# hila-chefer/Transformer-Explainability

Measured on AMD Instinct MI355X. Metric: relevance maps/sec (ViT-B/16 224^2, batch 64 per GPU, generate_LRP transformer_attribution), higher is better.
Workload: dtype f32 (3xbf16 split operands, 6 products, fp32 accumulate)

## Files before the change

### include/te_relprop.h

```cpp
#ifndef TE_RELPROP_H
#define TE_RELPROP_H

#include <stddef.h>
#include <stdint.h>

#ifdef __cplusplus
extern "C" {
#endif

typedef void* te_stream_t;
typedef uint16_t te_bf16_t;

enum {
  TE_OK = 0,
  TE_ERR_INVALID_ARG = -1,
  TE_ERR_WORKSPACE = -2,
  TE_ERR_UNSUPPORTED = -3,
  TE_ERR_NO_DEVICE = -4
};

enum { TE_VARIANT_OURS = 0, TE_VARIANT_LRP = 1, TE_IMPL_SIMPLE = 0x100 };

enum { TE_ROLLOUT_NORMALISE = 1, TE_ROLLOUT_CLS_FIXUP = 2, TE_ROLLOUT_ROW0 = 4 };

// ... 46 lines not shown
                       void* ws, size_t ws_bytes, te_stream_t stream);

size_t te_add_relprop_deferred_workspace_bytes(int64_t B, int64_t n);
int te_add_relprop_deferred_f32(const float* R, const float* X0, const float* X1, float* a, float* b, float* fac,
                                int64_t B, int64_t n, int64_t x1_batch_stride,
                                void* ws, size_t ws_bytes, te_stream_t stream);

size_t te_add_bcast_relprop_workspace_bytes(int64_t B, int64_t H, int64_t N);
int te_add_bcast_relprop_f32(const float* R, const float* X0, const float* mask, float* out0,
                             float* out1, int64_t B, int64_t H, int64_t N, int variant,
                             void* ws, size_t ws_bytes, te_stream_t stream);

int te_add_bcast_relprop_deferred_f32(const float* R, const float* X0, const float* mask, float* a, float* out1,
                                      float* fac, int64_t B, int64_t H, int64_t N,
                                      void* ws, size_t ws_bytes, te_stream_t stream);

int te_clone_relprop_f32(const float* R0, const float* R1, const float* R2, const float* X,
                         float* out, int64_t n, te_stream_t stream);

int te_clone_relprop_scaled_f32(const float* R0, const float* s0, int64_t s0_stride,
                                const float* R1, const float* s1, int64_t s1_stride,
                                const float* R2, const float* s2, int64_t s2_stride,
                                const float* X, float* out, int64_t B, int64_t n, te_stream_t stream);

int te_index_select_relprop_f32(const float* R, const float* X, float* out,
                                int64_t B, int64_t N, int64_t C, int64_t index, te_stream_t stream);

int te_gradcam_headmean_f32(const float* grad, const float* cam, float* out,
                            int64_t B, int64_t H, int64_t N, te_stream_t stream);

size_t te_rollout_workspace_bytes(int64_t L, int64_t B, int64_t N);
size_t te_rollout_row0_workspace_bytes(int64_t B, int64_t N);
int te_rollout_f32(const float* cams, int64_t L, int64_t start_layer, int64_t B, int64_t N,
                   int flags, float* joint, void* ws, size_t ws_bytes, te_stream_t stream);

#define TE_X6_TILE_AUTO 0
#define TE_X6_TILE_128 1
#define TE_X6_TILE_256 2
#define TE_X6_TILE_128x128 3
#define TE_X6_TEST_DROP_HANDOVER 0x200
#define TE_X6_WHOLE_TILES 0x10000
#define TE_X6_TEST_SMALL_GRID 0x4000
#define TE_X6_X_PLANES_SIGNED 0x20000
#define TE_X6_TILE_Z_SHIFT 10
#define TE_X6_TILE_C_SHIFT 12
#define TE_X6_PHASE_SPLIT 4
// ... 51 lines not shown
int te_attention_strided_supported(int64_t N, int64_t D);
size_t te_attention_backward_strided_workspace_bytes(int64_t B, int64_t H, int64_t N);
int te_attention_forward_strided_f32(const float* q, int64_t q_sb, int64_t q_sh, int64_t q_sn,
                                     const float* k, int64_t k_sb, int64_t k_sh, int64_t k_sn,
                                     const float* v, int64_t v_sb, int64_t v_sh, int64_t v_sn,
                                     const float* mask, float* z_qk, float* x_scaled, float* attn,
                                     float* out, int64_t o_sb, int64_t o_sh, int64_t o_sn,
                                     int64_t B, int64_t H, int64_t N, int64_t D, float scale, te_stream_t stream);
int te_attention_backward_strided_f32(const float* d_out, int64_t do_sb, int64_t do_sh, int64_t do_sn,
                                      const float* out, int64_t o_sb, int64_t o_sh, int64_t o_sn,
                                      const float* q, int64_t q_sb, int64_t q_sh, int64_t q_sn,
                                      const float* k, int64_t k_sb, int64_t k_sh, int64_t k_sn,
                                      const float* v, int64_t v_sb, int64_t v_sh, int64_t v_sn,
                                      const float* attn, float* d_attn,
                                      float* d_q, int64_t dq_sb, int64_t dq_sh, int64_t dq_sn,
                                      float* d_k, int64_t dk_sb, int64_t dk_sh, int64_t dk_sn,
                                      float* d_v, int64_t dv_sb, int64_t dv_sh, int64_t dv_sn,
                                      int64_t B, int64_t H, int64_t N, int64_t D, float scale, int need_qk,
                                      void* ws, size_t ws_bytes, te_stream_t stream);

int te_layernorm_supported(int64_t C);
int te_layernorm_forward_f32(const float* x, const float* weight, const float* bias, float* y, float* mean, float* rstd,
                             int64_t T, int64_t C, float eps, te_stream_t stream);
int te_layernorm_backward_f32(const float* dy, const float* x, const float* weight, const float* mean, const float* rstd,
                              const float* add, float* dx, int64_t T, int64_t C, te_stream_t stream);
int te_gelu_forward_f32(const float* x, float* y, int64_t n, te_stream_t stream);
int te_gelu_backward_f32(const float* dy, const float* x, float* dx, int64_t n, te_stream_t stream);

int te_heatmap_f32(const float* maps, float* heat, float* fg_mask, int64_t B, int64_t g, int64_t scale,
                   int normalise, te_stream_t stream);

size_t te_seg_metrics_workspace_bytes(int64_t B, int64_t H, int64_t W);
int te_seg_metrics_f32(const float* heat, const float* fg_mask, const int64_t* labels, int64_t* counts, double* ap,
                       double* f1, int64_t B, int64_t H, int64_t W, void* ws, size_t ws_bytes, te_stream_t stream);

#define TE_MAPSIM_SSIM 1
size_t te_map_similarity_workspace_bytes(int64_t B, int64_t n);
int te_map_similarity_f32(const float* a, const float* b, int64_t* rank_sums, double* sim, int64_t B, int64_t n, int64_t H,
                          int64_t W, int flags, double data_range, void* ws, size_t ws_bytes, te_stream_t stream);

#define TE_RATIONALE_MAX_KS 16
#define TE_RATIONALE_CLAMP 1
size_t te_rationale_metrics_workspace_bytes(int64_t B, int64_t N, int64_t Wmax);
int te_rationale_metrics_f32(const float* scores, const int32_t* word_ids, const uint8_t* truth, float* word_scores,
                             int32_t* n_words, int32_t* order, int32_t* counts, double* soft, int64_t B, int64_t N,
                             int64_t Wmax, const int64_t* ks, int64_t n_ks, int flags, void* ws, size_t ws_bytes,
// ... 212 lines not shown
```

### transformer-explainability_amd/csrc/te_api.hip

```cpp
#include "te_common.h"

#include <string.h>

extern "C" int te_version(void) { return 800;  }

#ifndef TE_BUILD_ID
#define TE_BUILD_ID "unstamped"
#endif
extern "C" const char* te_build_id(void) { return TE_BUILD_ID; }

extern "C" const char* te_status_string(int status) {
  switch (status) {
    case TE_OK: return "ok";
    case TE_ERR_INVALID_ARG: return "invalid argument";
    case TE_ERR_WORKSPACE: return "workspace missing, misaligned or too small";
    case TE_ERR_UNSUPPORTED: return "shape not supported by the gfx950 kernels";
    case TE_ERR_NO_DEVICE: return "no gfx950 device visible";
    default: break;
  }
  if (status > 0) return hipGetErrorString((hipError_t)status);
  return "unknown status";
}

extern "C" int te_device_check(void) {
  int n = 0;
  if (hipGetDeviceCount(&n) != hipSuccess || n <= 0) return TE_ERR_NO_DEVICE;
  for (int d = 0; d < n; ++d) {
// ... 7 lines not shown
```

### transformer-explainability_amd/csrc/te_elementwise.hip

```cpp
#include <stdlib.h>

#include "te_common.h"

namespace {

constexpr int kThreads = 256;


template <typename V>
__device__ __forceinline__ V ld(const float* p) { return *reinterpret_cast<const V*>(p); }
template <typename V>
__device__ __forceinline__ void st(float* p, V v) { *reinterpret_cast<V*>(p) = v; }

__device__ __forceinline__ float ldx(const float* p) { return *p; }
__device__ __forceinline__ float ldx(const te_bf16_t* p) { return __uint_as_float((unsigned)*p << 16); }
template <typename V>
__device__ __forceinline__ V ldx4(const float* p) { return ld<V>(p); }
template <typename V>
__device__ __forceinline__ V ldx4(const te_bf16_t* p) { return V{ldx(p), ldx(p + 1), ldx(p + 2), ldx(p + 3)}; }
static inline bool vec_aligned(const float* p) { return te_aligned16(p); }
static inline bool vec_aligned(const te_bf16_t*) { return true; }

template <int VEC, typename TX>
__global__ __launch_bounds__(kThreads) void add_sums_kernel(
// ... 354 lines not shown
  const TX* x_ = X + b * n;
  float* o = out + b * n;
  const int64_t stride = (int64_t)gridDim.x * kThreads * VEC;
  for (int64_t i = ((int64_t)blockIdx.x * kThreads + threadIdx.x) * VEC; i < n; i += stride) {
    if constexpr (VEC == 4) {
      const f32x4 x = ldx4<f32x4>(x_ + i), a = ld<f32x4>(r0 + i), bq = ld<f32x4>(r1 + i);
      f32x4 c = {0.f, 0.f, 0.f, 0.f};
      if constexpr (NUM == 3) c = ld<f32x4>(r2 + i);
      f32x4 ov;
#pragma unroll
      for (int e = 0; e < 4; ++e) {
        const float ra = s0 ? a[e] * f0 : a[e], rb = s1 ? bq[e] * f1 : bq[e];
        float s = te_sd(ra, x[e]) + te_sd(rb, x[e]);
        if constexpr (NUM == 3) s = s + te_sd(s2 ? c[e] * f2 : c[e], x[e]);
        ov[e] = x[e] * s;
      }
      st<f32x4>(o + i, ov);
    } else {
      const float x = ldx(x_ + i);
      float s = te_sd(s0 ? r0[i] * f0 : r0[i], x) + te_sd(s1 ? r1[i] * f1 : r1[i], x);
      if constexpr (NUM == 3) s = s + te_sd(s2 ? r2[i] * f2 : r2[i], x);
      o[i] = x * s;
    }
  }
}

template <typename TX>
__global__ __launch_bounds__(kThreads) void index_select_kernel(
    const float* __restrict__ R, const TX* __restrict__ X, float* __restrict__ out,
    int64_t B, int64_t N, int64_t C, int64_t index) {
  const int64_t total = B * N * C;
  const int64_t stride = (int64_t)gridDim.x * kThreads;
  for (int64_t i = (int64_t)blockIdx.x * kThreads + threadIdx.x; i < total; i += stride) {
    const int64_t c = i % C;
    const int64_t nrow = (i / C) % N;
    const int64_t b = i / (C * N);
    float v = 0.0f;
    if (nrow == index) {
      const float x = ldx(X + i);
      v = x * te_sd(R[b * C + c], x);
    }
    out[i] = v;
  }
}

template <int VEC, typename TG>
// ... 385 lines not shown
                                    float* out, int64_t n, te_stream_t stream_) {
  return clone_relprop(R0, R1, R2, X, out, n, stream_);
}

extern "C" int te_clone_relprop_bf16(const float* R0, const float* R1, const float* R2, const te_bf16_t* X, float* out,
                                     int64_t n, te_stream_t stream_) {
  return clone_relprop(R0, R1, R2, X, out, n, stream_);
}

extern "C" int te_clone_relprop_scaled_f32(const float* R0, const float* s0, int64_t s0_stride, const float* R1,
                                           const float* s1, int64_t s1_stride, const float* R2, const float* s2,
                                           int64_t s2_stride, const float* X, float* out, int64_t B, int64_t n,
                                           te_stream_t stream_) {
  return clone_relprop_scaled(R0, s0, s0_stride, R1, s1, s1_stride, R2, s2, s2_stride, X, out, B, n, stream_);
}

extern "C" int te_clone_relprop_scaled_bf16(const float* R0, const float* s0, int64_t s0_stride, const float* R1,
                                            const float* s1, int64_t s1_stride, const float* R2, const float* s2,
                                            int64_t s2_stride, const te_bf16_t* X, float* out, int64_t B, int64_t n,
                                            te_stream_t stream_) {
  return clone_relprop_scaled(R0, s0, s0_stride, R1, s1, s1_stride, R2, s2, s2_stride, X, out, B, n, stream_);
}

namespace {
template <typename TX>
int index_select_relprop(const float* R, const TX* X, float* out, int64_t B, int64_t N, int64_t C, int64_t index,
                         te_stream_t stream_) {
  if (!R || !X || !out || B <= 0 || N <= 0 || C <= 0 || index < 0 || index >= N)
    return TE_ERR_INVALID_ARG;
  hipStream_t stream = (hipStream_t)stream_;
  int64_t blocks = te_ceil_div(B * N * C, (int64_t)kThreads * 4);
  if (blocks > 4096) blocks = 4096;
  index_select_kernel<<<dim3((unsigned)blocks), dim3(kThreads), 0, stream>>>(R, X, out, B, N, C, index);
  TE_RETURN_IF_LAUNCH_FAILED();
  return TE_OK;
}

}

extern "C" int te_index_select_relprop_f32(const float* R, const float* X, float* out, int64_t B,
                                           int64_t N, int64_t C, int64_t index, te_stream_t stream_) {
  return index_select_relprop(R, X, out, B, N, C, index, stream_);
}

extern "C" int te_index_select_relprop_bf16(const float* R, const te_bf16_t* X, float* out, int64_t B, int64_t N,
                                            int64_t C, int64_t index, te_stream_t stream_) {
// ... 57 lines not shown
```

### transformer-explainability_amd/csrc/te_norm_act.hip

```cpp
#include "te_common.h"

namespace {

constexpr int kThreads = 256;
constexpr int kRowsPerBlock = kThreads / 64;
constexpr int kMaxChunks = 8;

__device__ __forceinline__ float wave_sum_all(float v) {
#pragma unroll
  for (int off = 32; off > 0; off >>= 1) v = v + __shfl_xor(v, off, 64);
  return v;
}

template <int NV>
__global__ __launch_bounds__(kThreads) void ln_fwd_kernel(const float* __restrict__ x, const float* __restrict__ w,
                                                          const float* __restrict__ b, float* __restrict__ y,
                                                          float* __restrict__ mean, float* __restrict__ rstd, int64_t T,
                                                          int C, float eps) {
  const int lane = threadIdx.x & 63;
  const int64_t row = (int64_t)blockIdx.x * kRowsPerBlock + (threadIdx.x >> 6);
  if (row >= T) return;
  const int nc = C >> 2;
  const float* xr = x + row * C;
  f32x4 v[NV];
  float s = 0.0f;
#pragma unroll
  for (int i = 0; i < NV; ++i) {
    const int c = lane + 64 * i;
    v[i] = f32x4{0.f, 0.f, 0.f, 0.f};
    if (c < nc) v[i] = *reinterpret_cast<const f32x4*>(xr + (c << 2));
    s = s + ((v[i][0] + v[i][1]) + (v[i][2] + v[i][3]));
  }
  const float m = wave_sum_all(s) / (float)C;
  float q = 0.0f;
#pragma unroll
  for (int i = 0; i < NV; ++i) {
    const int c = lane + 64 * i;
    if (c < nc) {
#pragma unroll
      for (int e = 0; e < 4; ++e) {
        const float d = v[i][e] - m;
        q = q + d * d;
      }
    }
  }
  const float r = 1.0f / sqrtf(wave_sum_all(q) / (float)C + eps);
  float* yr = y + row * C;
#pragma unroll
  for (int i = 0; i < NV; ++i) {
    const int c = lane + 64 * i;
    if (c < nc) {
      const f32x4 wv = *reinterpret_cast<const f32x4*>(w + (c << 2));
      const f32x4 bv = b ? *reinterpret_cast<const f32x4*>(b + (c << 2)) : f32x4{0.f, 0.f, 0.f, 0.f};
// ... 96 lines not shown
  }
  return TE_OK;
}

}

extern "C" int te_layernorm_supported(int64_t C) { return (C >= 4 && C % 4 == 0 && C <= 64 * 4 * kMaxChunks) ? 1 : 0; }

extern "C" int te_layernorm_forward_f32(const float* x, const float* weight, const float* bias, float* y, float* mean,
                                        float* rstd, int64_t T, int64_t C, float eps, te_stream_t stream_) {
  if (!x || !weight || !y || !mean || !rstd || T <= 0) return TE_ERR_INVALID_ARG;
  if (!te_layernorm_supported(C) || (T + kRowsPerBlock - 1) / kRowsPerBlock > 0x7fffffff) return TE_ERR_UNSUPPORTED;
  if (!te_aligned16(x) || !te_aligned16(weight) || !te_aligned16(y) || (bias && !te_aligned16(bias))) return TE_ERR_UNSUPPORTED;
  hipStream_t stream = (hipStream_t)stream_;
  const dim3 grid((unsigned)((T + kRowsPerBlock - 1) / kRowsPerBlock)), blk(kThreads);
  const int rc = for_chunks(C, [&](auto nv) {
    ln_fwd_kernel<decltype(nv)::value><<<grid, blk, 0, stream>>>(x, weight, bias, y, mean, rstd, T, (int)C, eps);
  });
  if (rc != TE_OK) return rc;
  TE_RETURN_IF_LAUNCH_FAILED();
  return TE_OK;
}

extern "C" int te_layernorm_backward_f32(const float* dy, const float* x, const float* weight, const float* mean,
                                         const float* rstd, const float* add, float* dx, int64_t T, int64_t C,
                                         te_stream_t stream_) {
  if (!dy || !x || !weight || !mean || !rstd || !dx || T <= 0) return TE_ERR_INVALID_ARG;
  if (!te_layernorm_supported(C) || (T + kRowsPerBlock - 1) / kRowsPerBlock > 0x7fffffff) return TE_ERR_UNSUPPORTED;
  if (!te_aligned16(dy) || !te_aligned16(x) || !te_aligned16(weight) || !te_aligned16(dx) || (add && !te_aligned16(add)))
    return TE_ERR_UNSUPPORTED;
  hipStream_t stream = (hipStream_t)stream_;
  const dim3 grid((unsigned)((T + kRowsPerBlock - 1) / kRowsPerBlock)), blk(kThreads);
  const int rc = for_chunks(C, [&](auto nv) {
    ln_bwd_kernel<decltype(nv)::value><<<grid, blk, 0, stream>>>(dy, x, weight, mean, rstd, add, dx, T, (int)C);
  });
  if (rc != TE_OK) return rc;
  TE_RETURN_IF_LAUNCH_FAILED();
  return TE_OK;
}

extern "C" int te_gelu_forward_f32(const float* x, float* y, int64_t n, te_stream_t stream_) {
  if (!x || !y || n <= 0) return TE_ERR_INVALID_ARG;
  if (n % 4 || !te_aligned16(x) || !te_aligned16(y) || n / 4 / kThreads > 0x7ffffffe) return TE_ERR_UNSUPPORTED;
  const int64_t n4 = n / 4;
  gelu_fwd_kernel<<<dim3((unsigned)((n4 + kThreads - 1) / kThreads)), dim3(kThreads), 0, (hipStream_t)stream_>>>(x, y, n4);
  TE_RETURN_IF_LAUNCH_FAILED();
// ... 12 lines not shown
```

### transformer-explainability_amd/ops.py

```python
from __future__ import annotations

import contextlib
import os
from typing import Optional, Sequence, Tuple

import torch

from . import _lib
from ._lib import (TE_HEADMEAN_CLAMP, TE_HEADMEAN_ROW0, TE_IMPL_SIMPLE, TE_RATIONALE_CLAMP, TE_ROLLOUT_CLS_FIXUP,
                   TE_ROLLOUT_NORMALISE, TE_ROLLOUT_ROW0, TE_VARIANT_LRP, TE_VARIANT_OURS)
from ._lib import (TE_X6_PHASE_C, TE_X6_PHASE_SPLIT, TE_X6_PHASE_Z, TE_X6_TEST_DROP_HANDOVER,
                   TE_X6_TEST_SMALL_GRID, TE_X6_TILE_C_SHIFT, TE_X6_TILE_Z_SHIFT, TE_X6_WHOLE_TILES, TE_X6_X_PLANES_SIGNED)

Tensor = torch.Tensor
_VARIANTS = {"ours": TE_VARIANT_OURS, "lrp": TE_VARIANT_LRP}

FORCE_SIMPLE = False
KERNEL_TIMER = None
_NULL = contextlib.nullcontext()


def _timed(name: str, flops: float = 0.0, nbytes: float = 0.0):
    return _NULL if KERNEL_TIMER is None else KERNEL_TIMER(name, float(flops), float(nbytes))

# ... 805 lines not shown
                   "te_attention_backward_f32")
    return d_attn, d_qkv


def layernorm_supported(x: Tensor) -> bool:
    return (x.is_cuda and x.dtype == torch.float32 and x.dim() >= 2
            and bool(_lib.load().te_layernorm_supported(int(x.shape[-1]))))


def layernorm_forward(x: Tensor, weight: Tensor, bias: Optional[Tensor], eps: float) -> Tuple[Tensor, Tensor, Tensor]:
    x = _c(x)
    C = x.shape[-1]
    T = x.numel() // C
    y = torch.empty_like(x)
    mean = torch.empty((T,), dtype=torch.float32, device=x.device)
    rstd = torch.empty((T,), dtype=torch.float32, device=x.device)
    with _on_device(x) as lib, _timed("layernorm_forward", 0.0, 4.0 * 2 * T * C):
        _lib.check(lib.te_layernorm_forward_f32(_ptr(x), _ptr(_c(weight)), _ptr(_c(bias)) if bias is not None else None,
                                                _ptr(y), _ptr(mean), _ptr(rstd), T, C, float(eps), _stream(x)),
                   "te_layernorm_forward_f32")
    return y, mean, rstd


def layernorm_backward(dy: Tensor, x: Tensor, weight: Tensor, mean: Tensor, rstd: Tensor,
                       add: Optional[Tensor] = None) -> Tensor:
    dy, x = _c(dy), _c(x)
    C = x.shape[-1]
    T = x.numel() // C
    dx = torch.empty_like(x)
    with _on_device(x) as lib, _timed("layernorm_backward", 0.0, 4.0 * (3 + (add is not None)) * T * C):
        _lib.check(lib.te_layernorm_backward_f32(_ptr(dy), _ptr(x), _ptr(_c(weight)), _ptr(mean), _ptr(rstd),
                                                 _ptr(_c(add)) if add is not None else None, _ptr(dx), T, C, _stream(x)),
                   "te_layernorm_backward_f32")
    return dx


def gelu_forward(x: Tensor) -> Tensor:
    x = _c(x)
    y = torch.empty_like(x)
    with _on_device(x) as lib, _timed("gelu_forward", 0.0, 4.0 * 2 * x.numel()):
        _lib.check(lib.te_gelu_forward_f32(_ptr(x), _ptr(y), x.numel(), _stream(x)), "te_gelu_forward_f32")
    return y


X6_FUSE_GELU = os.environ.get("TE_X6_FUSE_GELU", "1") not in ("", "0")

# ... 124 lines not shown
    X = _c16(X) if bf else _c(X)
    sfx = "bf16" if bf else "f32"
    pairs = [_split_deferred(r) for r in Rs]
    Rs = [_c(r) for r, _ in pairs]
    scales = [sc for _, sc in pairs]
    for r in Rs:
        if r.numel() != X.numel():
            raise _lib.TeError("Clone.relprop: relevance / input size mismatch")
    out = torch.empty(X.shape, dtype=torch.float32, device=X.device)
    nb = 4.0 * X.numel() * (len(Rs) + 1) + X.element_size() * X.numel()
    if any(sc is not None for sc in scales):
        B = X.shape[0]
        sp = [(None, 0) if sc is None else (sc.data_ptr(), sc.stride(0)) for sc in scales] + [(None, 0)]
        with _on_device(X) as lib, _timed("clone", 0.0, nb):
            _lib.check(getattr(lib, "te_clone_relprop_scaled_" + sfx)(
                _ptr(Rs[0]), sp[0][0], sp[0][1], _ptr(Rs[1]), sp[1][0], sp[1][1], _ptr(Rs[2]) if len(Rs) == 3 else None,
                sp[2][0], sp[2][1], _ptr(X), _ptr(out), B, X.numel() // B, _stream(X)), "te_clone_relprop_scaled_" + sfx)
        return out
    with _on_device(X) as lib, _timed("clone", 0.0, nb):
        _lib.check(getattr(lib, "te_clone_relprop_" + sfx)(_ptr(Rs[0]), _ptr(Rs[1]), _ptr(Rs[2]) if len(Rs) == 3 else None,
                                                           _ptr(X), _ptr(out), X.numel(), _stream(X)),
                   "te_clone_relprop_" + sfx)
    return out


def index_select_relprop(R: Tensor, X: Tensor, index: int) -> Tensor:
    if _any_f64(R, X):
        return index_select_relprop_f64(R, X, index)
    bf = _is_bf16(X)
    X = _c16(X) if bf else _c(X)
    B, N, C = X.shape
    R = _c(R).reshape(B, C)
    out = torch.empty(X.shape, dtype=torch.float32, device=X.device)
    sfx = "bf16" if bf else "f32"
    with _on_device(X) as lib:
        _lib.check(getattr(lib, "te_index_select_relprop_" + sfx)(_ptr(R), _ptr(X), _ptr(out), B, N, C, int(index),
                                                                   _stream(X)), "te_index_select_relprop_" + sfx)
    return out


def gradcam_headmean(grad: Tensor, cam: Tensor, out: Optional[Tensor] = None) -> Tensor:
    if _any_f64(grad, cam, out):
        return gradcam_headmean_f64(grad, cam, out)
    bf = _is_bf16(grad)
    grad, cam = (_c16(grad) if bf else _c(grad)), _c(cam)
    B, H, N, _ = cam.shape
# ... 1289 lines not shown
```

### transformer-explainability_amd/producers.py

```python
from __future__ import annotations

import torch

from . import ops


def usable(x: torch.Tensor) -> bool:
    return ops.USE_FUSED_PRODUCERS and torch.is_tensor(x) and ops.layernorm_supported(x)


def gelu_usable(x: torch.Tensor) -> bool:
    return (ops.USE_FUSED_PRODUCERS and torch.is_tensor(x) and x.is_cuda and x.dtype == torch.float32
            and x.numel() > 0 and x.numel() % 4 == 0)


def norm_usable(x: torch.Tensor, norm) -> bool:
    return (usable(x) and not norm.training and getattr(norm, "weight", None) is not None
            and tuple(norm.normalized_shape) == (x.shape[-1],))


class _LayerNorm(torch.autograd.Function):
    @staticmethod
    def forward(ctx, x, weight, bias, eps):
        y, mean, rstd = ops.layernorm_forward(x, weight, bias, eps)
        ctx.save_for_backward(x, weight, mean, rstd)
        return y

    @staticmethod
    def backward(ctx, dy):
        x, weight, mean, rstd = ctx.saved_tensors
        return ops.layernorm_backward(dy, x, weight, mean, rstd), None, None, None


class _ResidualLayerNorm(torch.autograd.Function):

    @staticmethod
    def forward(ctx, x, weight, bias, eps):
        y, mean, rstd = ops.layernorm_forward(x, weight, bias, eps)
        ctx.save_for_backward(x, weight, mean, rstd)
        return x.view_as(x), y

    @staticmethod
    def backward(ctx, d_bypass, dy):
        x, weight, mean, rstd = ctx.saved_tensors
        if dy is None:
            return d_bypass, None, None, None
        return ops.layernorm_backward(dy, x, weight, mean, rstd, add=d_bypass), None, None, None


class _Gelu(torch.autograd.Function):

    @staticmethod
    def forward(ctx, x, feeds, source):
        ctx.save_for_backward(x)
        ctx.source = source
        if feeds is not None:
            y, xs, xa = ops.gelu_forward_planes(x, not ops.X6_SIGNED_PLANES)
            ops.post_x_planes(feeds, y, xs, xa)
            return y
        return ops.gelu_forward(x)

    @staticmethod
    def backward(ctx, dy):
        (x,) = ctx.saved_tensors
        if ctx.source is not None:
            return ops.post_dy_planes(ctx.source, ops.gelu_backward_planes(dy, x), x), None, None
        return ops.gelu_backward(dy, x), None, None


class _Linear(torch.autograd.Function):
# ... 66 lines not shown
```

### transformer-explainability_amd/rules.py

```python
from __future__ import annotations

import contextlib

import torch
import torch.nn as nn

from . import ops

__all__ = ['forward_hook', 'Clone', 'Add', 'Cat', 'ReLU', 'GELU', 'Dropout', 'BatchNorm2d', 'Linear', 'MaxPool2d',
           'AdaptiveAvgPool2d', 'AvgPool2d', 'Conv2d', 'Sequential', 'safe_divide', 'einsum', 'Softmax',
           'IndexSelect', 'LayerNorm', 'AddEye', 'Tanh', 'MatMul', 'Mul']


def safe_divide(a, b):
    den = b.clamp(min=1e-9) + b.clamp(max=1e-9)
    den = den + den.eq(0).type(den.type()) * 1e-9
    return a / den * b.ne(0).type(b.type())


def forward_hook(self, input, output):
    if type(input[0]) in (list, tuple):
        self.X = [i.detach() for i in input[0]]
    else:
        self.X = input[0].detach()
# ... 233 lines not shown
    go = heads(ops._c(G_o))
    d_attn = torch.matmul(go, heads(v).transpose(-1, -2))
    heads(d_v).copy_(torch.matmul(attn.transpose(-1, -2), go))
    d_s = attn * (d_attn - (d_attn * attn).sum(dim=-1, keepdim=True))
    heads(d_q).copy_(torch.matmul(d_s, heads(k)) * scale)
    heads(d_k).copy_(torch.matmul(d_s.transpose(-1, -2), heads(q)) * scale)


class Clone(RelProp):

    def forward(self, input, num):
        self.__setattr__('num', num)
        return [input for _ in range(num)]

    def relprop(self, R, alpha):
        return ops.clone_relprop(list(R), self.X)

    def attnlrp(self, G, eps):
        G = list(G)
        out = G[0] + G[1]
        for g in G[2:]:
            out += g
        return out


class IndexSelect(RelProp):

    def forward(self, inputs, dim, indices):
        self.__setattr__('dim', dim)
        self.__setattr__('indices', indices)
        if not torch.is_tensor(indices):
            self._index_host = int(indices)
        elif indices.numel() == 1 and (not indices.is_cuda or getattr(self, "_index_src", None) is not indices
                                       or getattr(self, "_index_version", None) != indices._version):
            if not (indices.is_cuda and torch.cuda.is_current_stream_capturing()):
                self._index_host = int(indices)
                self._index_src = indices
                self._index_version = indices._version
        return torch.index_select(inputs, dim, indices.reshape(-1) if torch.is_tensor(indices) else indices)

    def relprop(self, R, alpha):
        idx = self.indices
        if self.dim != 1 or self.X.dim() != 3 or (torch.is_tensor(idx) and idx.numel() != 1):
            raise NotImplementedError("IndexSelect.relprop: only dim=1 with a single index is accelerated")
        host = getattr(self, "_index_host", None)
        if host is None or (torch.is_tensor(idx) and (getattr(self, "_index_src", idx) is not idx
# ... 105 lines not shown
```

### transformer-explainability_amd/vit.py

```python
from __future__ import annotations

import torch
import torch.nn as nn

from . import methods, ops, producers
from . import rules as R_ours

__all__ = ["VisionTransformer", "vit_base_patch16_224", "vit_large_patch16_224", "deit_base_patch16_224",
           "compute_rollout_attention", "make_vit_module"]


def compute_rollout_attention(all_layer_matrices, start_layer=0):
    return ops.rollout(torch.stack(list(all_layer_matrices), 0), start_layer=start_layer, normalise=False)


def tail_full(model, cam, **kwargs):
    cam, _ = model.add.relprop(cam, **kwargs)
    cam = model.patch_embed.relprop(cam[:, 1:], **kwargs)
    return cam.sum(dim=1)


def tail_rollout(model, start_layer=0):
    mats = [blk.attn.get_attn_cam().clamp(min=0).mean(dim=1) for blk in model.blocks]
    return compute_rollout_attention(mats, start_layer=start_layer)[:, 0, 1:]
# ... 253 lines not shown
            if self.head_mask is not None:
                raise ops._lib.TeError("Attention.attnlrp: head_mask is not implemented for AttnLRP")
            G_o = self.proj.attnlrp(G, eps)
            B, N, C = G_o.shape
            qkv = self.qkv.Y.detach()
            d_qkv = torch.empty_like(qkv)
            third = lambda t, i: t[..., i * C:(i + 1) * C]
            R_ours.attention_attnlrp(G_o, third(qkv, 0), third(qkv, 1), third(qkv, 2), self.get_attn().detach(),
                                     self.num_heads, self.scale, third(d_qkv, 0), third(d_qkv, 1), third(d_qkv, 2))
            return self.qkv.attnlrp(ops.alrp_scale3(d_qkv), eps)

    class Block(nn.Module):
        def __init__(self, dim, num_heads, mlp_ratio=4., qkv_bias=False, drop=0., attn_drop=0., norm_eps=1e-6):
            super().__init__()
            self.norm1 = L.LayerNorm(dim, eps=norm_eps)
            self.attn = Attention(dim, num_heads=num_heads, qkv_bias=qkv_bias, attn_drop=attn_drop, proj_drop=drop)
            self.norm2 = L.LayerNorm(dim, eps=norm_eps)
            self.mlp = Mlp(in_features=dim, hidden_features=int(dim * mlp_ratio), drop=drop)
            self.add1 = L.Add()
            self.add2 = L.Add()
            self.clone1 = L.Clone()
            self.clone2 = L.Clone()

        def forward(self, x, head_mask=None):
            x1, n = self._clone_norm(self.clone1, self.norm1, x)
            x = self.add1([x1, self.attn(n) if head_mask is None else self.attn(n, head_mask)])
            x1, n = self._clone_norm(self.clone2, self.norm2, x)
            return self.add2([x1, self.mlp(n)])

        @staticmethod
        def _clone_norm(clone, norm, x):
            if producers.norm_usable(x, norm):
                x1, n = producers.residual_layer_norm(x, norm)
                clone.X, clone.num = x.detach(), 2
                norm.X, norm.Y = clone.X, n
                return x1, n
            x1, x2 = clone(x, 2)
            return x1, norm(x2)

        def relprop(self, cam, **kwargs):
            cam1, cam2 = self.add2.relprop(cam, deferred=True, **kwargs)
            cam2 = self.mlp.relprop(cam2, **kwargs)
            cam = self.clone2.relprop((cam1, cam2), **kwargs)
            cam1, cam2 = self.add1.relprop(cam, deferred=True, **kwargs)
            cam2 = self.attn.relprop(cam2, **kwargs)
            return self.clone1.relprop((cam1, cam2), **kwargs)

        def attnlrp(self, G, eps):
            Gd = self.add2.attnlrp(G, eps)
            G = self.clone2.attnlrp((Gd, self.norm2.attnlrp(self.mlp.attnlrp(Gd, eps), eps)), eps)
            Gd = self.add1.attnlrp(G, eps)
            return self.clone1.attnlrp((Gd, self.norm1.attnlrp(self.attn.attnlrp(Gd, eps), eps)), eps)

        def relprop_cls_only(self, cam_cls, **kwargs):
            alpha = kwargs.get("alpha", 1)
            var = self.add2.variant
            cls = lambda t: t[:, :1]
            dfr = ops.USE_DEFERRED_ADD
            c1, c2 = ops.add_relprop(cam_cls, cls(self.add2.X[0]), cls(self.add2.X[1]), variant=var, deferred=dfr)
            c2 = R_ours.linear_rule(self.mlp.fc2, c2, alpha, cls, var)
            c2 = R_ours.linear_rule(self.mlp.fc1, c2, alpha, cls, var)
            cam = ops.clone_relprop((c1, c2), cls(self.clone2.X))
            c1, c2 = ops.add_relprop(cam, cls(self.add1.X[0]), cls(self.add1.X[1]), variant=var, deferred=dfr)
            c2 = R_ours.linear_rule(self.attn.proj, c2, alpha, cls, var)
            if isinstance(c1, ops.Deferred):
                c1 = c1.materialise()
            B, N, C = self.clone1.X.shape
            dense = torch.zeros((2, B, N, C), dtype=c2.dtype, device=c2.device)
            dense[0, :, 0] = c1[:, 0]
            dense[1, :, 0] = c2[:, 0]
            cam2 = self.attn.relprop_after_proj(dense[1], **kwargs)
            return self.clone1.relprop((dense[0], cam2), **kwargs)

    class PatchEmbed(nn.Module):
        def __init__(self, img_size=224, patch_size=16, in_chans=3, embed_dim=768):
            super().__init__()
            img_size = (img_size, img_size) if isinstance(img_size, int) else tuple(img_size)
            patch_size = (patch_size, patch_size) if isinstance(patch_size, int) else tuple(patch_size)
            self.img_size, self.patch_size = img_size, patch_size
            self.num_patches = (img_size[1] // patch_size[1]) * (img_size[0] // patch_size[0])
            self.proj = L.Conv2d(in_chans, embed_dim, kernel_size=patch_size, stride=patch_size)

        def forward(self, x):
            B, C, Hh, Ww = x.shape
            assert Hh == self.img_size[0] and Ww == self.img_size[1], \
                f"Input image size ({Hh}*{Ww}) doesn't match model ({self.img_size[0]}*{self.img_size[1]})."
            return self.proj(x).flatten(2).transpose(1, 2)

        def relprop(self, cam, **kwargs):
            cam = cam.unflatten(1, (self.img_size[0] // self.patch_size[0], self.img_size[1] // self.patch_size[1]))
            return self.proj.relprop(cam.permute(0, 3, 1, 2), **kwargs)

    class VisionTransformer(nn.Module):
        default_method = "transformer_attribution" if L.RelProp.variant == "ours" else "grad"

# ... 34 lines not shown
                    nn.init.constant_(m.bias, 0)
            elif isinstance(m, nn.LayerNorm):
                nn.init.constant_(m.bias, 0)
                nn.init.constant_(m.weight, 1.0)

        @property
        def no_weight_decay(self):
            return {'pos_embed', 'cls_token'}

        def get_head_mask(self, head_mask, batch_size=None):
            return R_ours.expand_head_mask(head_mask, len(self.blocks), self.blocks[0].attn.num_heads, self.pos_embed.dtype,
                                           batch_size, self.pos_embed.device)

        def forward(self, x, register_hook=False, head_mask=None):
            B = x.shape[0]
            head_mask = self.get_head_mask(head_mask, B)
            with (ops.stock_forward() if torch.is_tensor(head_mask) else ops._NULL):
                x = self.patch_embed(x)
                x = torch.cat((self.cls_token.expand(B, -1, -1), x), dim=1)
                x = self.add([x, self.pos_embed])
                if x.requires_grad:
                    x.register_hook(self.save_inp_grad)
                for blk, hm in zip(self.blocks, head_mask):
                    x = blk(x) if hm is None else blk(x, hm)
                x = self.norm(x)
                x = self.pool(x, dim=1, indices=self._cls_index).squeeze(1)
                return self.head(x)

        def relprop(self, cam=None, method=None, is_ablation=False, start_layer=0, **kwargs):
            if method is None:
                method = self.default_method
            several = not isinstance(method, str)
            wanted = tuple(method) if several else (method,)
            if "full" in wanted and ops._is_f64(cam):
                raise ops._lib.TeError(f"{ops.DTYPES_MSG}; method='full' (the z^B patch rule) is not implemented for "
                                       "torch.float64 relevance: run it on a float32 or bfloat16 model")
            if several:
                prune = self.prune_below_start_layer and methods.prunable(wanted, methods.LRP_NEEDS)
            else:
                prune = self.prune_below_start_layer and method in methods.SINGLE_CALL_PRUNED
            try:
                with L.stop_after_attn_cam(self.blocks[start_layer].attn if prune else None):
                    cam = self.head.relprop(cam, **kwargs)
                    if self.exploit_cls_sparsity and isinstance(self.head, nn.Linear):
                        cam = ops.index_select_relprop(cam.unsqueeze(1), self.pool.X[:, :1], 0)
                        cam = self.blocks[-1].relprop_cls_only(cam, **kwargs)
                        rest = list(self.blocks)[:-1]
                    else:
                        cam = self.pool.relprop(cam.unsqueeze(1), **kwargs)
                        rest = list(self.blocks)
                    for blk in reversed(rest):
                        cam = blk.relprop(cam, **kwargs)
            except L.StopRelprop:
                cam = None

            hook = getattr(self, "_before_tail", None)
            if hook is not None:
                hook()

            maps = {m: relprop_tail(self, m, cam, is_ablation, start_layer, prune, **kwargs) for m in wanted}
            return maps if several else maps[method]

        def attnlrp(self, seed, eps=1e-6):
            G = self.head.attnlrp(seed, eps)
            G = self.norm.attnlrp(self.pool.attnlrp(G, eps), eps)
            for blk in reversed(self.blocks):
                G = blk.attnlrp(G, eps)
            return ops.alrp_token_relevance(self.add.X[0], G, skip_first=True)

    def vit_base_patch16_224(pretrained=False, **kwargs):
        model = VisionTransformer(patch_size=16, embed_dim=768, depth=12, num_heads=12, mlp_ratio=4, qkv_bias=True,
                                  **kwargs)
        if pretrained:
            load_pretrained_weights(model, PRETRAINED_URLS["vit_base_patch16_224"], patch_size=16)
        return model
# ... 28 lines not shown
```

Before: 1027.

## Fuse residual add with layernorm forward and clone+add relprop seams

Adds a fused add+layernorm forward kernel so each residual sum is written once and normalised in the same pass, and defers block outputs as pending tuples so that fusion can happen across block boundaries. In the relevance pass, the Clone relprop at each residual seam is folded into the following deferred Add relprop through a new kernel that computes both outputs and the per-sample factors in one sweep. This removes intermediate tensor round-trips and kernel launches at every block seam. In exchange it adds pending-object plumbing and version/alias checks, with fallbacks to the original path when those checks fail.

```diff
diff --git a/include/te_relprop.h b/include/te_relprop.h
--- a/include/te_relprop.h
+++ b/include/te_relprop.h
@@ -92,6 +92,12 @@
                                 const float* R1, const float* s1, int64_t s1_stride,
                                 const float* R2, const float* s2, int64_t s2_stride,
                                 const float* X, float* out, int64_t B, int64_t n, te_stream_t stream);
+
+int te_clone_add_relprop_deferred_f32(const float* R0, const float* s0, int64_t s0_stride,
+                                      const float* R1, const float* s1, int64_t s1_stride,
+                                      const float* X0, const float* X1, int64_t x1_batch_stride,
+                                      float* a, float* b, float* fac, int64_t B, int64_t n,
+                                      void* ws, size_t ws_bytes, te_stream_t stream);
 
 int te_index_select_relprop_f32(const float* R, const float* X, float* out,
                                 int64_t B, int64_t N, int64_t C, int64_t index, te_stream_t stream);
@@ -189,6 +195,8 @@
 int te_layernorm_supported(int64_t C);
 int te_layernorm_forward_f32(const float* x, const float* weight, const float* bias, float* y, float* mean, float* rstd,
                              int64_t T, int64_t C, float eps, te_stream_t stream);
+int te_add_layernorm_forward_f32(const float* a, const float* b, const float* weight, const float* bias, float* sum,
+                                 float* y, float* mean, float* rstd, int64_t T, int64_t C, float eps, te_stream_t stream);
 int te_layernorm_backward_f32(const float* dy, const float* x, const float* weight, const float* mean, const float* rstd,
                               const float* add, float* dx, int64_t T, int64_t C, te_stream_t stream);
 int te_gelu_forward_f32(const float* x, float* y, int64_t n, te_stream_t stream);
diff --git a/transformer-explainability_amd/csrc/te_api.hip b/transformer-explainability_amd/csrc/te_api.hip
--- a/transformer-explainability_amd/csrc/te_api.hip
+++ b/transformer-explainability_amd/csrc/te_api.hip
@@ -2,7 +2,7 @@
 
 #include <string.h>
 
-extern "C" int te_version(void) { return 800;  }
+extern "C" int te_version(void) { return 801;  }
 
 #ifndef TE_BUILD_ID
 #define TE_BUILD_ID "unstamped"
diff --git a/transformer-explainability_amd/csrc/te_elementwise.hip b/transformer-explainability_amd/csrc/te_elementwise.hip
--- a/transformer-explainability_amd/csrc/te_elementwise.hip
+++ b/transformer-explainability_amd/csrc/te_elementwise.hip
@@ -400,6 +400,65 @@
       if constexpr (NUM == 3) s = s + te_sd(s2 ? r2[i] * f2 : r2[i], x);
       o[i] = x * s;
     }
+  }
+}
+
+template <int VEC, typename TX>
+__global__ __launch_bounds__(kThreads) void clone_add_deferred_kernel(
+    const float* __restrict__ R0, const float* __restrict__ s0, int64_t s0_stride, const float* __restrict__ R1,
+    const float* __restrict__ s1, int64_t s1_stride, const TX* __restrict__ X0, const TX* __restrict__ X1,
+    float* __restrict__ a_out, float* __restrict__ b_out, double* __restrict__ partial, int64_t n, int64_t x1_bs,
+    int64_t chunk) {
+  __shared__ double smem[3 * (kThreads / 64)];
+  const int64_t b = blockIdx.y;
+  const float f0 = s0 ? s0[b * s0_stride] : 1.0f, f1 = s1 ? s1[b * s1_stride] : 1.0f;
+  const int64_t start = (int64_t)blockIdx.x * chunk;
+  const int64_t end = min(n, start + chunk);
+  const float* r0 = R0 + b * n;
+  const float* r1 = R1 + b * n;
+  const TX* x0 = X0 + b * n;
+  const TX* x1 = X1 + b * x1_bs;
+  float* o0 = a_out + b * n;
+  float* o1 = b_out + b * n;
+  double sa = 0.0, sb = 0.0, sr = 0.0;
+  for (int64_t i = start + (int64_t)threadIdx.x * VEC; i < end; i += (int64_t)kThreads * VEC) {
+    if constexpr (VEC == 4) {
+      const f32x4 pv = ld<f32x4>(r0 + i), qv = ld<f32x4>(r1 + i), av = ldx4<f32x4>(x0 + i), bv = ldx4<f32x4>(x1 + i);
+      f32x4 oa, ob;
+#pragma unroll
+      for (int e = 0; e < 4; ++e) {
+        const float x = av[e] + bv[e];
+        const float ra = s0 ? pv[e] * f0 : pv[e], rb = s1 ? qv[e] * f1 : qv[e];
+        const float rv = x * (te_sd(ra, x) + te_sd(rb, x));
+        const float s = te_sd(rv, x);
+        oa[e] = av[e] * s;
+        ob[e] = bv[e] * s;
+        sa += (double)oa[e];
+        sb += (double)ob[e];
+        sr += (double)rv;
+      }
+      st<f32x4>(o0 + i, oa);
+      st<f32x4>(o1 + i, ob);
+    } else {
+      const float av = ldx(x0 + i), bv = ldx(x1 + i);
+      const float x = av + bv;
+      const float ra = s0 ? r0[i] * f0 : r0[i], rb = s1 ? r1[i] * f1 : r1[i];
+      const float rv = x * (te_sd(ra, x) + te_sd(rb, x));
+      const float s = te_sd(rv, x);
+      const float a = av * s, bb = bv * s;
+      o0[i] = a;
+      o1[i] = bb;
+      sa += (double)a;
+      sb += (double)bb;
+      sr += (double)rv;
+    }
+  }
+  te_block_sum3(sa, sb, sr, smem);
+  if (threadIdx.x == 0) {
+    double* p = partial + (b * gridDim.x + blockIdx.x) * 3;
+    p[0] = sa;
+    p[1] = sb;
+    p[2] = sr;
   }
 }
 
@@ -831,6 +890,33 @@
   return clone_relprop_scaled(R0, s0, s0_stride, R1, s1, s1_stride, R2, s2, s2_stride, X, out, B, n, stream_);
 }
 
+extern "C" int te_clone_add_relprop_deferred_f32(const float* R0, const float* s0, int64_t s0_stride, const float* R1,
+                                                 const float* s1, int64_t s1_stride, const float* X0, const float* X1,
+                                                 int64_t x1_batch_stride, float* a, float* b, float* fac, int64_t B,
+                                                 int64_t n, void* ws, size_t ws_bytes, te_stream_t stream_) {
+  if (!R0 || !R1 || !X0 || !X1 || !a || !b || !fac || B <= 0 || n <= 0) return TE_ERR_INVALID_ARG;
+  if (x1_batch_stride != 0 && x1_batch_stride != n) return TE_ERR_INVALID_ARG;
+  if (B > 65535) return TE_ERR_UNSUPPORTED;
+  if (!ws || ws_bytes < te_add_relprop_workspace_bytes(B, n)) return TE_ERR_WORKSPACE;
+  hipStream_t stream = (hipStream_t)stream_;
+  const bool vec = (n % 4 == 0) && te_aligned16(R0) && te_aligned16(R1) && te_aligned16(X0) && te_aligned16(X1) &&
+                   te_aligned16(a) && te_aligned16(b);
+  const int bps = pick_blocks_per_sample(B, n);
+  int64_t chunk = te_ceil_div(n, bps);
+  chunk = te_ceil_div(chunk, 4) * 4;
+  dim3 grid(bps, (unsigned)B), block(kThreads);
+  double* partial = (double*)ws;
+  if (vec)
+    clone_add_deferred_kernel<4><<<grid, block, 0, stream>>>(R0, s0, s0_stride, R1, s1, s1_stride, X0, X1, a, b, partial,
+                                                             n, x1_batch_stride, chunk);
+  else
+    clone_add_deferred_kernel<1><<<grid, block, 0, stream>>>(R0, s0, s0_stride, R1, s1, s1_stride, X0, X1, a, b, partial,
+                                                             n, x1_batch_stride, chunk);
+  add_factors_kernel<<<dim3((unsigned)B), dim3(64), 0, stream>>>(partial, fac, bps);
+  TE_RETURN_IF_LAUNCH_FAILED();
+  return TE_OK;
+}
+
 namespace {
 template <typename TX>
 int index_select_relprop(const float* R, const TX* X, float* out, int64_t B, int64_t N, int64_t C, int64_t index,
diff --git a/transformer-explainability_amd/csrc/te_norm_act.hip b/transformer-explainability_amd/csrc/te_norm_act.hip
--- a/transformer-explainability_amd/csrc/te_norm_act.hip
+++ b/transformer-explainability_amd/csrc/te_norm_act.hip
@@ -29,6 +29,67 @@
     const int c = lane + 64 * i;
     v[i] = f32x4{0.f, 0.f, 0.f, 0.f};
     if (c < nc) v[i] = *reinterpret_cast<const f32x4*>(xr + (c << 2));
+    s = s + ((v[i][0] + v[i][1]) + (v[i][2] + v[i][3]));
+  }
+  const float m = wave_sum_all(s) / (float)C;
+  float q = 0.0f;
+#pragma unroll
+  for (int i = 0; i < NV; ++i) {
+    const int c = lane + 64 * i;
+    if (c < nc) {
+#pragma unroll
+      for (int e = 0; e < 4; ++e) {
+        const float d = v[i][e] - m;
+        q = q + d * d;
+      }
+    }
+  }
+  const float r = 1.0f / sqrtf(wave_sum_all(q) / (float)C + eps);
+  float* yr = y + row * C;
+#pragma unroll
+  for (int i = 0; i < NV; ++i) {
+    const int c = lane + 64 * i;
+    if (c < nc) {
+      const f32x4 wv = *reinterpret_cast<const f32x4*>(w + (c << 2));
+      const f32x4 bv = b ? *reinterpret_cast<const f32x4*>(b + (c << 2)) : f32x4{0.f, 0.f, 0.f, 0.f};
+      f32x4 o;
+#pragma unroll
+      for (int e = 0; e < 4; ++e) o[e] = ((v[i][e] - m) * r) * wv[e] + bv[e];
+      __builtin_nontemporal_store(o, reinterpret_cast<f32x4*>(yr + (c << 2)));
+    }
+  }
+  if (lane == 0) {
+    mean[row] = m;
+    rstd[row] = r;
+  }
+}
+
+template <int NV>
+__global__ __launch_bounds__(kThreads) void add_ln_fwd_kernel(const float* __restrict__ a, const float* __restrict__ b2,
+                                                              const float* __restrict__ w, const float* __restrict__ b,
+                                                              float* __restrict__ sum, float* __restrict__ y,
+                                                              float* __restrict__ mean, float* __restrict__ rstd,
+                                                              int64_t T, int C, float eps) {
+  const int lane = threadIdx.x & 63;
+  const int64_t row = (int64_t)blockIdx.x * kRowsPerBlock + (threadIdx.x >> 6);
+  if (row >= T) return;
+  const int nc = C >> 2;
+  const float* ar = a + row * C;
+  const float* br = b2 + row * C;
+  float* sr = sum + row * C;
+  f32x4 v[NV];
+  float s = 0.0f;
+#pragma unroll
+  for (int i = 0; i < NV; ++i) {
+    const int c = lane + 64 * i;
+    v[i] = f32x4{0.f, 0.f, 0.f, 0.f};
+    if (c < nc) {
+      const f32x4 av = *reinterpret_cast<const f32x4*>(ar + (c << 2));
+      const f32x4 bv = *reinterpret_cast<const f32x4*>(br + (c << 2));
+#pragma unroll
+      for (int e = 0; e < 4; ++e) v[i][e] = av[e] + bv[e];
+      *reinterpret_cast<f32x4*>(sr + (c << 2)) = v[i];
+    }
     s = s + ((v[i][0] + v[i][1]) + (v[i][2] + v[i][3]));
   }
   const float m = wave_sum_all(s) / (float)C;
@@ -171,6 +232,24 @@
   return TE_OK;
 }
 
+extern "C" int te_add_layernorm_forward_f32(const float* a, const float* b, const float* weight, const float* bias,
+                                            float* sum, float* y, float* mean, float* rstd, int64_t T, int64_t C, float eps,
+                                            te_stream_t stream_) {
+  if (!a || !b || !weight || !sum || !y || !mean || !rstd || T <= 0) return TE_ERR_INVALID_ARG;
+  if (!te_layernorm_supported(C) || (T + kRowsPerBlock - 1) / kRowsPerBlock > 0x7fffffff) return TE_ERR_UNSUPPORTED;
+  if (!te_aligned16(a) || !te_aligned16(b) || !te_aligned16(weight) || !te_aligned16(sum) || !te_aligned16(y) ||
+      (bias && !te_aligned16(bias)))
+    return TE_ERR_UNSUPPORTED;
+  hipStream_t stream = (hipStream_t)stream_;
+  const dim3 grid((unsigned)((T + kRowsPerBlock - 1) / kRowsPerBlock)), blk(kThreads);
+  const int rc = for_chunks(C, [&](auto nv) {
+    add_ln_fwd_kernel<decltype(nv)::value><<<grid, blk, 0, stream>>>(a, b, weight, bias, sum, y, mean, rstd, T, (int)C, eps);
+  });
+  if (rc != TE_OK) return rc;
+  TE_RETURN_IF_LAUNCH_FAILED();
+  return TE_OK;
+}
+
 extern "C" int te_layernorm_backward_f32(const float* dy, const float* x, const float* weight, const float* mean,
                                          const float* rstd, const float* add, float* dx, int64_t T, int64_t C,
                                          te_stream_t stream_) {
diff --git a/transformer-explainability_amd/ops.py b/transformer-explainability_amd/ops.py
--- a/transformer-explainability_amd/ops.py
+++ b/transformer-explainability_amd/ops.py
@@ -851,6 +851,24 @@
     return y, mean, rstd
 
 
+def add_layernorm_forward(a: Tensor, b: Tensor, weight: Tensor, bias: Optional[Tensor],
+                          eps: float) -> Tuple[Tensor, Tensor, Tensor, Tensor]:
+    a, b = _c(a), _c(b)
+    if a.shape != b.shape:
+        raise _lib.TeError(f"add_layernorm_forward: operand shapes {tuple(a.shape)} and {tuple(b.shape)} differ")
+    C = a.shape[-1]
+    T = a.numel() // C
+    total, y = torch.empty_like(a), torch.empty_like(a)
+    mean = torch.empty((T,), dtype=torch.float32, device=a.device)
+    rstd = torch.empty((T,), dtype=torch.float32, device=a.device)
+    with _on_device(a) as lib, _timed("add_layernorm_forward", 0.0, 4.0 * 4 * T * C):
+        _lib.check(lib.te_add_layernorm_forward_f32(_ptr(a), _ptr(b), _ptr(_c(weight)),
+                                                    _ptr(_c(bias)) if bias is not None else None, _ptr(total), _ptr(y),
+                                                    _ptr(mean), _ptr(rstd), T, C, float(eps), _stream(a)),
+                   "te_add_layernorm_forward_f32")
+    return total, y, mean, rstd
+
+
 def layernorm_backward(dy: Tensor, x: Tensor, weight: Tensor, mean: Tensor, rstd: Tensor,
                        add: Optional[Tensor] = None) -> Tensor:
     dy, x = _c(dy), _c(x)
@@ -1021,6 +1039,38 @@
                                                            _ptr(X), _ptr(out), X.numel(), _stream(X)),
                    "te_clone_relprop_" + sfx)
     return out
+
+
+FUSE_RESIDUAL_SEAMS = True
+
+
+def clone_add_relprop(Rs: Sequence, X0: Tensor, X1: Tensor):
+    if len(Rs) != 2:
+        raise _lib.TeError(f"clone_add_relprop takes the 2 aliases of a residual Clone, got {len(Rs)}")
+    X0, X1 = _c(X0), _c(X1)
+    B = X0.shape[0]
+    n = X0[0].numel()
+    if X1.shape == X0.shape:
+        x1_bs = n
+    elif X1.shape[0] == 1 and X1.shape[1:] == X0.shape[1:]:
+        x1_bs = 0
+    else:
+        raise _lib.TeError(f"clone_add_relprop: unsupported operand shapes {tuple(X0.shape)} + {tuple(X1.shape)}")
+    pairs = [_split_deferred(r) for r in Rs]
+    Rt = [_c(r) for r, _ in pairs]
+    for r in Rt:
+        if r.numel() != X0.numel():
+            raise _lib.TeError("clone_add_relprop: relevance / input size mismatch")
+    sp = [(None, 0) if sc is None else (sc.data_ptr(), sc.stride(0)) for _, sc in pairs]
+    out0, out1 = torch.empty_like(X0), torch.empty_like(X0)
+    fac = torch.empty((B, 2), dtype=torch.float32, device=X0.device)
+    with _on_device(X0) as lib, _timed("clone_add_deferred", 0.0, 4.0 * B * (5 * n + (n if x1_bs else n / B))):
+        ws = _ws(lib.te_add_relprop_deferred_workspace_bytes(B, n), X0)
+        _lib.check(lib.te_clone_add_relprop_deferred_f32(_ptr(Rt[0]), sp[0][0], sp[0][1], _ptr(Rt[1]), sp[1][0], sp[1][1],
+                                                         _ptr(X0), _ptr(X1), x1_bs, _ptr(out0), _ptr(out1), _ptr(fac), B,
+                                                         n, _ptr(ws), ws.numel(), _stream(X0)),
+                   "te_clone_add_relprop_deferred_f32")
+    return Deferred(out0, fac[:, 0]), Deferred(out1, fac[:, 1])
 
 
 def index_select_relprop(R: Tensor, X: Tensor, index: int) -> Tensor:
diff --git a/transformer-explainability_amd/producers.py b/transformer-explainability_amd/producers.py
--- a/transformer-explainability_amd/producers.py
+++ b/transformer-explainability_amd/producers.py
@@ -46,6 +46,32 @@
         if dy is None:
             return d_bypass, None, None, None
         return ops.layernorm_backward(dy, x, weight, mean, rstd, add=d_bypass), None, None, None
+
+
+class _AddResidualLayerNorm(torch.autograd.Function):
+
+    @staticmethod
+    def forward(ctx, a, b, weight, bias, eps):
+        total, y, mean, rstd = ops.add_layernorm_forward(a, b, weight, bias, eps)
+        ctx.save_for_backward(total, weight, mean, rstd)
+        ctx.set_materialize_grads(False)
+        return total, y
+
+    @staticmethod
+    def backward(ctx, d_total, dy):
+        total, weight, mean, rstd = ctx.saved_tensors
+        d = d_total if dy is None else ops.layernorm_backward(dy, total, weight, mean, rstd, add=d_total)
+        return d, d, None, None, None
+
+
+def add_norm_usable(a, b, norm) -> bool:
+    return (ops.FUSE_RESIDUAL_SEAMS and torch.is_tensor(a) and torch.is_tensor(b) and a.shape == b.shape
+            and a.dtype == b.dtype and a.device == b.device and a.is_contiguous() and b.is_contiguous()
+            and norm_usable(a, norm))
+
+
+def add_residual_layer_norm(a, b, norm):
+    return _AddResidualLayerNorm.apply(a, b, _d(norm.weight), _d(norm.bias), norm.eps)
 
 
 class _Gelu(torch.autograd.Function):
diff --git a/transformer-explainability_amd/rules.py b/transformer-explainability_amd/rules.py
--- a/transformer-explainability_amd/rules.py
+++ b/transformer-explainability_amd/rules.py
@@ -279,6 +279,47 @@
         for g in G[2:]:
             out += g
         return out
+
+
+class PendingClone:
+    __slots__ = ("Rs", "clone")
+
+    def __init__(self, Rs, clone):
+        self.Rs, self.clone = tuple(Rs), clone
+
+    def resolve(self, **kwargs):
+        return self.clone.relprop(self.Rs, **kwargs)
+
+
+def on_device(t) -> bool:
+    return t.is_cuda
+
+
+def seam_fusable(clone, add, Rs=None) -> bool:
+    if not (ops.FUSE_RESIDUAL_SEAMS and ops.USE_DEFERRED_ADD and isinstance(clone, Clone) and isinstance(add, Add)):
+        return False
+    X, Y, ab = getattr(clone, "X", None), getattr(add, "Y", None), getattr(add, "X", None)
+    if not (torch.is_tensor(X) and torch.is_tensor(Y) and isinstance(ab, (list, tuple)) and len(ab) == 2):
+        return False
+    if getattr(clone, "num", None) != 2 or (Rs is not None and len(Rs) != 2):
+        return False
+    if ops._variant(add.variant) != ops.TE_VARIANT_OURS:
+        return False
+    if not (X.data_ptr() == Y.data_ptr() and X.shape == Y.shape and X.stride() == Y.stride()
+            and X._version == Y._version == getattr(add, "_y_version", None)):
+        return False
+    a, b = ab
+    tensors = [X, a, b] + [r.t if isinstance(r, ops.Deferred) else r for r in (Rs or ())]
+    return (a.shape == b.shape == X.shape
+            and all(torch.is_tensor(t) and t.dtype == torch.float32 and on_device(t) for t in tensors))
+
+
+def add_after_clone(add, R, deferred=True, **kwargs):
+    if isinstance(R, PendingClone):
+        if deferred and seam_fusable(R.clone, add, R.Rs):
+            return list(ops.clone_add_relprop(R.Rs, add.X[0], add.X[1]))
+        R = R.resolve(**kwargs)
+    return add.relprop(R, deferred=deferred, **kwargs)
 
 
 class IndexSelect(RelProp):
diff --git a/transformer-explainability_amd/vit.py b/transformer-explainability_amd/vit.py
--- a/transformer-explainability_amd/vit.py
+++ b/transformer-explainability_amd/vit.py
@@ -299,29 +299,45 @@
             self.clone1 = L.Clone()
             self.clone2 = L.Clone()
 
-        def forward(self, x, head_mask=None):
+        def forward(self, x, head_mask=None, pending=False):
             x1, n = self._clone_norm(self.clone1, self.norm1, x)
-            x = self.add1([x1, self.attn(n) if head_mask is None else self.attn(n, head_mask)])
+            x = (self.add1, x1, self.attn(n) if head_mask is None else self.attn(n, head_mask))
             x1, n = self._clone_norm(self.clone2, self.norm2, x)
-            return self.add2([x1, self.mlp(n)])
+            x = (self.add2, x1, self.mlp(n))
+            return x if pending else x[0]([x[1], x[2]])
+
+        @staticmethod
+        def add_norm(x, norm):
+            if not isinstance(x, tuple):
+                return x, None
+            add, a, b = x
+            if producers.add_norm_usable(a, b, norm):
+                x, n = producers.add_residual_layer_norm(a, b, norm)
+                R_ours.forward_hook(add, ([a, b],), x)
+                return x, n
+            return add([a, b]), None
 
         @staticmethod
         def _clone_norm(clone, norm, x):
-            if producers.norm_usable(x, norm):
+            x, n = Block.add_norm(x, norm)
+            if n is not None:
+                x1 = x
+            elif producers.norm_usable(x, norm):
                 x1, n = producers.residual_layer_norm(x, norm)
-                clone.X, clone.num = x.detach(), 2
-                norm.X, norm.Y = clone.X, n
-                return x1, n
-            x1, x2 = clone(x, 2)
-            return x1, norm(x2)
-
-        def relprop(self, cam, **kwargs):
-            cam1, cam2 = self.add2.relprop(cam, deferred=True, **kwargs)
+            else:
+                x1, x2 = clone(x, 2)
+                return x1, norm(x2)
+            clone.X, clone.num = x.detach(), 2
+            norm.X, norm.Y = clone.X, n
+            return x1, n
+
+        def relprop(self, cam, pending=False, **kwargs):
+            cam1, cam2 = R_ours.add_after_clone(self.add2, cam, **kwargs)
             cam2 = self.mlp.relprop(cam2, **kwargs)
-            cam = self.clone2.relprop((cam1, cam2), **kwargs)
-            cam1, cam2 = self.add1.relprop(cam, deferred=True, **kwargs)
+            cam1, cam2 = R_ours.add_after_clone(self.add1, R_ours.PendingClone((cam1, cam2), self.clone2), **kwargs)
             cam2 = self.attn.relprop(cam2, **kwargs)
-            return self.clone1.relprop((cam1, cam2), **kwargs)
+            out = R_ours.PendingClone((cam1, cam2), self.clone1)
+            return out if pending else out.resolve(**kwargs)
 
         def attnlrp(self, G, eps):
             Gd = self.add2.attnlrp(G, eps)
@@ -329,7 +345,7 @@
             Gd = self.add1.attnlrp(G, eps)
             return self.clone1.attnlrp((Gd, self.norm1.attnlrp(self.attn.attnlrp(Gd, eps), eps)), eps)
 
-        def relprop_cls_only(self, cam_cls, **kwargs):
+        def relprop_cls_only(self, cam_cls, pending=False, **kwargs):
             alpha = kwargs.get("alpha", 1)
             var = self.add2.variant
             cls = lambda t: t[:, :1]
@@ -337,8 +353,11 @@
             c1, c2 = ops.add_relprop(cam_cls, cls(self.add2.X[0]), cls(self.add2.X[1]), variant=var, deferred=dfr)
             c2 = R_ours.linear_rule(self.mlp.fc2, c2, alpha, cls, var)
             c2 = R_ours.linear_rule(self.mlp.fc1, c2, alpha, cls, var)
-            cam = ops.clone_relprop((c1, c2), cls(self.clone2.X))
-            c1, c2 = ops.add_relprop(cam, cls(self.add1.X[0]), cls(self.add1.X[1]), variant=var, deferred=dfr)
+            if dfr and R_ours.seam_fusable(self.clone2, self.add1, (c1, c2)):
+                c1, c2 = ops.clone_add_relprop((c1, c2), cls(self.add1.X[0]), cls(self.add1.X[1]))
+            else:
+                cam = ops.clone_relprop((c1, c2), cls(self.clone2.X))
+                c1, c2 = ops.add_relprop(cam, cls(self.add1.X[0]), cls(self.add1.X[1]), variant=var, deferred=dfr)
             c2 = R_ours.linear_rule(self.attn.proj, c2, alpha, cls, var)
             if isinstance(c1, ops.Deferred):
                 c1 = c1.materialise()
@@ -347,7 +366,8 @@
             dense[0, :, 0] = c1[:, 0]
             dense[1, :, 0] = c2[:, 0]
             cam2 = self.attn.relprop_after_proj(dense[1], **kwargs)
-            return self.clone1.relprop((dense[0], cam2), **kwargs)
+            out = R_ours.PendingClone((dense[0], cam2), self.clone1)
+            return out if pending else out.resolve(**kwargs)
 
     class PatchEmbed(nn.Module):
         def __init__(self, img_size=224, patch_size=16, in_chans=3, embed_dim=768):
@@ -428,8 +448,13 @@
                 if x.requires_grad:
                     x.register_hook(self.save_inp_grad)
                 for blk, hm in zip(self.blocks, head_mask):
-                    x = blk(x) if hm is None else blk(x, hm)
-                x = self.norm(x)
+                    x = blk(x, pending=True) if hm is None else blk(x, hm, pending=True)
+                x, n = Block.add_norm(x, self.norm)
+                if n is None:
+                    x = self.norm(x)
+                else:
+                    R_ours.forward_hook(self.norm, (x,), n)
+                    x = n
                 x = self.pool(x, dim=1, indices=self._cls_index).squeeze(1)
                 return self.head(x)
 
@@ -450,13 +475,15 @@
                     cam = self.head.relprop(cam, **kwargs)
                     if self.exploit_cls_sparsity and isinstance(self.head, nn.Linear):
                         cam = ops.index_select_relprop(cam.unsqueeze(1), self.pool.X[:, :1], 0)
-                        cam = self.blocks[-1].relprop_cls_only(cam, **kwargs)
+                        cam = self.blocks[-1].relprop_cls_only(cam, pending=True, **kwargs)
                         rest = list(self.blocks)[:-1]
                     else:
                         cam = self.pool.relprop(cam.unsqueeze(1), **kwargs)
                         rest = list(self.blocks)
                     for blk in reversed(rest):
-                        cam = blk.relprop(cam, **kwargs)
+                        cam = blk.relprop(cam, pending=True, **kwargs)
+                    if isinstance(cam, R_ours.PendingClone):
+                        cam = cam.resolve(**kwargs)
             except L.StopRelprop:
                 cam = None
 
```

Result: no change. 1034 (median of 6 runs) (+0.6%).
